# hellboywyh/pytorch-kaldi-CGS

Hardware: AMD Instinct MI355X
Metric: acoustic frames/sec (train) (higher is better)
Workload: dtype bf16; 1 GPU; TIMIT_baselines MLP 440-5x1024-{1928,48} (TIMIT_MLP_fmllr.cfg), batch_size_train=128, dropout 0.15, SGD body + RMSprop heads; global_batch=128, parallelism=dp1, chunk_frames_per_rank=225345

## Files before the change

### pytorch-kaldi-cgs_amd/csrc/pkc_gemm.hip

```cpp
#include "pkc_gemm_big.h"
#include "pkc_ops.h"
#include "pkc_optim.h"

namespace pkc {

typedef __attribute__((ext_vector_type(8))) __bf16 bf16x8;
typedef __attribute__((ext_vector_type(16))) float f32x16;

constexpr int BM = 64, BN = 64, BK = 32, NT = 256;

template <int PREC>
struct Lds;
template <>
struct Lds<PKC_PREC_FP32> {
  using T = float;
  static constexpr int LD = BK + 4;
  static constexpr int LO = 0;
  float a[BM * LD];
  float b[BN * LD];
};
template <>
struct Lds<PKC_PREC_BF16> {
  using T = __bf16;
  static constexpr int LD = BK + 8;
// ... 11 lines not shown
  __bf16 al[BM * LD];
  __bf16 bl[BN * LD];
};

template <typename T, int LO>
__device__ __forceinline__ void put(T* __restrict__ s, int i, float v) {
  const T hv = (T)v;
  s[i] = hv;
  if constexpr (LO > 0) s[i + LO] = (T)(v - (float)hv);
}

__device__ __forceinline__ int swz4(int row, int c4) { return (c4 + (row >> 2)) & 7; }

template <bool KC, bool VEC>
struct Stage {
  float v[8];
  __device__ __forceinline__ void load(const float* __restrict__ P, int64_t ld, int r0, int rmax,
                                       int k0, int kend) {
    const int t = threadIdx.x;
    if (VEC) {
#pragma unroll
      for (int i = 0; i < 2; ++i) {
        const int idx = t + NT * i;
        int r, k;
        if (KC) { r = idx >> 3; k = (idx & 7) * 4; }
        else { k = idx >> 4; r = (idx & 15) * 4; }
        const bool ok = (r0 + r < rmax) && (k0 + k < kend);
        const int rr = min(r0 + r, rmax - (KC ? 1 : 4));
        const int kk = min(k0 + k, kend - (KC ? 4 : 1));
        const float4 x = KC ? *reinterpret_cast<const float4*>(P + (int64_t)rr * ld + kk)
                            : *reinterpret_cast<const float4*>(P + (int64_t)kk * ld + rr);
        v[4 * i + 0] = ok ? x.x : 0.f;
        v[4 * i + 1] = ok ? x.y : 0.f;
        v[4 * i + 2] = ok ? x.z : 0.f;
        v[4 * i + 3] = ok ? x.w : 0.f;
      }
    } else {
#pragma unroll
      for (int i = 0; i < 8; ++i) {
        const int idx = t + NT * i;
        int r, k;
        if (KC) { r = idx >> 5; k = idx & 31; }
        else { k = idx >> 6; r = idx & 63; }
        const bool ok = (r0 + r < rmax) && (k0 + k < kend);
        const int rr = min(r0 + r, rmax - 1);
        const int kk = min(k0 + k, kend - 1);
        const float x = KC ? P[(int64_t)rr * ld + kk] : P[(int64_t)kk * ld + rr];
        v[i] = ok ? x : 0.f;
      }
    }
  }
  struct Base {
    const float* p[2];
    bool ok[2];
  };
  __device__ __forceinline__ static Base lane_base(const void* __restrict__ Pv, int64_t ld, int r0,
                                                   int rmax) {
    const float* P = reinterpret_cast<const float*>(Pv);
    const int t = threadIdx.x;
    Base b;
#pragma unroll
    for (int i = 0; i < 2; ++i) {
      const int r = KC ? (t >> 3) + 32 * i : (t & 15) * 4;
      const int rr = min(r0 + r, rmax - (KC ? 1 : 4));
      b.p[i] = KC ? P + (int64_t)rr * ld : P + rr;
      b.ok[i] = r0 + r < rmax;
    }
    return b;
  }
  __device__ __forceinline__ void load_at(const Base& b, int ld, int k0, int kend) {
    const int t = threadIdx.x;
#pragma unroll
    for (int i = 0; i < 2; ++i) {
      const int k = KC ? (t & 7) * 4 : (t >> 4) + 16 * i;
      const bool ok = b.ok[i] && (k0 + k < kend);
      const int kk = min(k0 + k, kend - (KC ? 4 : 1));
      const float4 x = KC ? *reinterpret_cast<const float4*>(b.p[i] + kk)
                          : *reinterpret_cast<const float4*>(b.p[i] + (int64_t)kk * ld);
      v[4 * i + 0] = ok ? x.x : 0.f;
      v[4 * i + 1] = ok ? x.y : 0.f;
      v[4 * i + 2] = ok ? x.z : 0.f;
      v[4 * i + 3] = ok ? x.w : 0.f;
    }
  }
  template <typename T, int LD, int LO = 0>
  __device__ __forceinline__ void store(T* __restrict__ s) const {
    const int t = threadIdx.x;
    if (VEC) {
#pragma unroll
      for (int i = 0; i < 2; ++i) {
        const int idx = t + NT * i;
        if (KC) {
          const int r = idx >> 3, k = (idx & 7) * 4;
#pragma unroll
          for (int j = 0; j < 4; ++j) put<T, LO>(s, r * LD + k + j, v[4 * i + j]);
        } else {
          const int k = idx >> 4, r = (idx & 15) * 4;
          if constexpr (sizeof(T) == 4) {
#pragma unroll
            for (int j = 0; j < 4; ++j)
              s[(r + j) * LD + 4 * swz4(r + j, k >> 2) + (k & 3)] = (T)v[4 * i + j];
          } else {
#pragma unroll
            for (int j = 0; j < 4; ++j) put<T, LO>(s, (r + j) * LD + k, v[4 * i + j]);
          }
        }
      }
    } else {
#pragma unroll
      for (int i = 0; i < 8; ++i) {
        const int idx = t + NT * i;
        if (KC) {
          const int r = idx >> 5, k = idx & 31;
          put<T, LO>(s, r * LD + k, v[i]);
        } else {
          const int k = idx >> 6, r = idx & 63;
          if constexpr (sizeof(T) == 4) s[r * LD + 4 * swz4(r, k >> 2) + (k & 3)] = (T)v[i];
          else put<T, LO>(s, r * LD + k, v[i]);
        }
      }
    }
  }
};

__device__ __forceinline__ int tr_off_s(int k, int c) { return 128 * k + 16 * (c ^ (((k >> 1) & 1) << 2)); }

__device__ __forceinline__ bf16x8 tr_frag_s(const char* __restrict__ s, int rb, int kb, int lane) {
  typedef short v4s __attribute__((ext_vector_type(4)));
  typedef short v8s __attribute__((ext_vector_type(8)));
  typedef __attribute__((address_space(3))) v4s lv4s;
  const int q = (lane & 15) >> 2, p = lane & 3;
  const int row = rb + 16 * ((lane >> 4) & 1) + 4 * p;
  const int k0 = kb + 8 * (lane >> 5) + q;
  const v4s lo = __builtin_amdgcn_ds_read_tr16_b64_v4i16(
      (lv4s*)(s + tr_off_s(k0, row >> 3) + 8 * (p & 1)));
  const v4s hi = __builtin_amdgcn_ds_read_tr16_b64_v4i16(
      (lv4s*)(s + tr_off_s(k0 + 4, row >> 3) + 8 * (p & 1)));
  const v8s w = __builtin_shufflevector(lo, hi, 0, 1, 2, 3, 4, 5, 6, 7);
  return __builtin_bit_cast(bf16x8, w);
}

__device__ __forceinline__ bf16x8 ld8h(const __bf16* p) { return *reinterpret_cast<const bf16x8*>(p); }
__device__ __forceinline__ bf16x8 zero8h() {
  bf16x8 z;
#pragma unroll
  for (int j = 0; j < 8; ++j) z[j] = (__bf16)0.f;
  return z;
}

template <bool KC, bool VEC>
struct StageH {
  bf16x8 v;
  __device__ __forceinline__ void load(const __bf16* __restrict__ P, int64_t ld, int r0, int rmax,
                                       int k0, int kend) {
    const int t = threadIdx.x;
    int r, k;
    if (KC) { r = t >> 2; k = (t & 3) * 8; }
    else { k = t >> 3; r = (t & 7) * 8; }
    if (VEC) {
      const bool ok = (r0 + r < rmax) && (k0 + k < kend);
      const int rr = min(r0 + r, rmax - (KC ? 1 : 8));
      const int kk = min(k0 + k, kend - (KC ? 8 : 1));
      const bf16x8 x = KC ? ld8h(P + (int64_t)rr * ld + kk) : ld8h(P + (int64_t)kk * ld + rr);
      v = ok ? x : zero8h();
    } else {
#pragma unroll
      for (int j = 0; j < 8; ++j) {
        const int rj = KC ? r : r + j, kj = KC ? k + j : k;
        const bool ok = (r0 + rj < rmax) && (k0 + kj < kend);
        const int rr = min(r0 + rj, rmax - 1), kk = min(k0 + kj, kend - 1);
        const __bf16 x = KC ? P[(int64_t)rr * ld + kk] : P[(int64_t)kk * ld + rr];
        v[j] = ok ? x : (__bf16)0.f;
      }
    }
  }
  struct Base {
    const __bf16* p;
    bool ok;
  };
  __device__ __forceinline__ static Base lane_base(const void* __restrict__ Pv, int64_t ld, int r0,
                                                   int rmax) {
    const __bf16* P = reinterpret_cast<const __bf16*>(Pv);
    const int t = threadIdx.x;
    const int r = KC ? t >> 2 : (t & 7) * 8;
    const int rr = min(r0 + r, rmax - (KC ? 1 : 8));
    return Base{KC ? P + (int64_t)rr * ld : P + rr, r0 + r < rmax};
  }
  __device__ __forceinline__ void load_at(const Base& b, int ld, int k0, int kend) {
    const int t = threadIdx.x;
    const int k = KC ? (t & 3) * 8 : t >> 3;
    const bool ok = b.ok && (k0 + k < kend);
    const int kk = min(k0 + k, kend - (KC ? 8 : 1));
    const bf16x8 x = KC ? ld8h(b.p + kk) : ld8h(b.p + (int64_t)kk * ld);
    v = ok ? x : zero8h();
  }
  template <typename T, int LD, int LO = 0>
  __device__ __forceinline__ void store(T* __restrict__ s) const {
    static_assert(LO == 0, "bf16-stored operands have no tail");
    const int t = threadIdx.x;
    if (KC) {
      const int r = t >> 2, k = (t & 3) * 8;
      *reinterpret_cast<bf16x8*>(&s[r * LD + k]) = v;
    } else {
      const int k = t >> 3, r = (t & 7) * 8;
      *reinterpret_cast<bf16x8*>(reinterpret_cast<char*>(s) + tr_off_s(k, r >> 3)) = v;
    }
  }
};

template <bool BIN, bool KC, bool VEC>
struct StageSel {
  using T = Stage<KC, VEC>;
  using E = float;
};
template <bool KC, bool VEC>
struct StageSel<true, KC, VEC> {
  using T = StageH<KC, VEC>;
  using E = __bf16;
};

template <int PREC, bool AKC, bool BKC, bool ATR = false, bool BTR = false>
__device__ __forceinline__ void mfma_tile(const Lds<PREC>& sm, int wm, int wn, int r, int h,
                                          f32x16& acc) {
  constexpr int LD = Lds<PREC>::LD;
  const int ra = wm * 32 + r, rb = wn * 32 + r;
  if constexpr (PREC == PKC_PREC_FP32) {
    const float4* pa = reinterpret_cast<const float4*>(&sm.a[ra * LD + 16 * h]);
    const float4* pb = reinterpret_cast<const float4*>(&sm.b[rb * LD + 16 * h]);
    float av[16], bv[16];
#pragma unroll
    for (int q = 0; q < 4; ++q) {
      float4 x, y;
      if constexpr (AKC) x = pa[q];
      else x = *reinterpret_cast<const float4*>(&sm.a[ra * LD + 4 * swz4(ra, 4 * h + q)]);
      if constexpr (BKC) y = pb[q];
      else y = *reinterpret_cast<const float4*>(&sm.b[rb * LD + 4 * swz4(rb, 4 * h + q)]);
      av[4 * q] = x.x; av[4 * q + 1] = x.y; av[4 * q + 2] = x.z; av[4 * q + 3] = x.w;
      bv[4 * q] = y.x; bv[4 * q + 1] = y.y; bv[4 * q + 2] = y.z; bv[4 * q + 3] = y.w;
    }
#pragma unroll
    for (int kk = 0; kk < 16; ++kk)
      acc = __builtin_amdgcn_mfma_f32_32x32x2f32(av[kk], bv[kk], acc, 0, 0, 0);
  } else if constexpr (PREC == PKC_PREC_BF16X3) {
#pragma unroll
    for (int t = 0; t < 2; ++t) {
      const int ia = (wm * 32 + r) * LD + 16 * t + 8 * h, ib = (wn * 32 + r) * LD + 16 * t + 8 * h;
      const bf16x8 av = *reinterpret_cast<const bf16x8*>(&sm.a[ia]);
      const bf16x8 bv = *reinterpret_cast<const bf16x8*>(&sm.b[ib]);
      const bf16x8 al = *reinterpret_cast<const bf16x8*>(&sm.al[ia]);
      const bf16x8 bl = *reinterpret_cast<const bf16x8*>(&sm.bl[ib]);
      acc = __builtin_amdgcn_mfma_f32_32x32x16_bf16(av, bl, acc, 0, 0, 0);
      acc = __builtin_amdgcn_mfma_f32_32x32x16_bf16(al, bv, acc, 0, 0, 0);
      acc = __builtin_amdgcn_mfma_f32_32x32x16_bf16(av, bv, acc, 0, 0, 0);
    }
  } else {
    const int lane = threadIdx.x & 63;
#pragma unroll
    for (int t = 0; t < 2; ++t) {
      bf16x8 av, bv;
      if constexpr (ATR) av = tr_frag_s(reinterpret_cast<const char*>(sm.a), wm * 32, 16 * t, lane);
      else av = *reinterpret_cast<const bf16x8*>(&sm.a[(wm * 32 + r) * LD + 16 * t + 8 * h]);
      if constexpr (BTR) bv = tr_frag_s(reinterpret_cast<const char*>(sm.b), wn * 32, 16 * t, lane);
      else bv = *reinterpret_cast<const bf16x8*>(&sm.b[(wn * 32 + r) * LD + 16 * t + 8 * h]);
      acc = __builtin_amdgcn_mfma_f32_32x32x16_bf16(av, bv, acc, 0, 0, 0);
    }
  }
}

template <int PREC>
__device__ __forceinline__ void tile_colstats64(const f32x16& acc, Lds<PREC>& sm, int m0, int n0,
                                                int by, int M, int N, int wm, int wn, int r, int h,
                                                const float* __restrict__ bias,
                                                float* __restrict__ part) {
  float* red = reinterpret_cast<float*>(&sm);
  const int nv = min(BM, M - m0);
  const int cl = wn * 32 + r;
  __syncthreads();
  float sum = 0.f;
#pragma unroll
  for (int reg = 0; reg < 16; ++reg) {
    const int rl = wm * 32 + (reg & 3) + 8 * (reg >> 2) + 4 * h;
    sum += rl < nv ? acc[reg] : 0.f;
  }
  sum += __shfl_xor(sum, 32);
  if (h == 0) red[wm * BN + cl] = sum;
  __syncthreads();
  const float mean = (red[cl] + red[BN + cl]) / (float)nv;
  float q = 0.f;
#pragma unroll
  for (int reg = 0; reg < 16; ++reg) {
    const int rl = wm * 32 + (reg & 3) + 8 * (reg >> 2) + 4 * h;
    const float d = acc[reg] - mean;
    q += rl < nv ? d * d : 0.f;
  }
  q += __shfl_xor(q, 32);
  if (h == 0) red[2 * BN + wm * BN + cl] = q;
  __syncthreads();
  const int col = n0 + cl;
  if (wm != 0 || h != 0 || col >= N) return;
  part[(int64_t)by * 2 * N + col] = mean + (bias ? bias[col] : 0.f);
  part[(int64_t)by * 2 * N + N + col] = red[2 * BN + cl] + red[3 * BN + cl];
}

template <int PREC, bool AKC, bool BKC, bool VEC, int DEPTH, bool BIN, bool STATS = false>
__device__ __forceinline__ void gemm_body(Lds<PREC>& sm, int bx, int by, int bz, int M, int N, int K,
                                          const void* __restrict__ Av, int64_t lda,
                                          const void* __restrict__ Bv, int64_t ldb,
                                          float* __restrict__ C, int64_t ldc, int kchunk,
                                          int64_t slab_stride, const float* __restrict__ bias = nullptr,
                                          float* __restrict__ part = nullptr) {
  using SA = typename StageSel<BIN, AKC, VEC>::T;
  using SB = typename StageSel<BIN, BKC, VEC>::T;
  const auto* A = reinterpret_cast<const typename StageSel<BIN, AKC, VEC>::E*>(Av);
  const auto* B = reinterpret_cast<const typename StageSel<BIN, BKC, VEC>::E*>(Bv);
  constexpr int LD = Lds<PREC>::LD;
  const int n0 = bx * BN, m0 = by * BM;
  const int kbeg = bz * kchunk;
  const int kend = min(K, kbeg + kchunk);
  const int lane = threadIdx.x & 63, wave = threadIdx.x >> 6;
  const int wm = wave >> 1, wn = wave & 1;
  const int r = lane & 31, h = lane >> 5;

  f32x16 acc;
#pragma unroll
  for (int i = 0; i < 16; ++i) acc[i] = 0.f;

  SA sa[DEPTH];
  SB sb[DEPTH];
  bool done = false;
  if constexpr (VEC) {
    const int nk = (kend - kbeg + BK - 1) / BK;
    if (kbeg < kend && nk <= DEPTH) {
      const typename SA::Base ab = SA::lane_base(A, lda, m0, M);
      const typename SB::Base bb = SB::lane_base(B, ldb, n0, N);
#pragma unroll
      for (int d = 0; d < DEPTH; ++d) {
        if (d >= nk) break;
        sa[d].load_at(ab, (int)lda, kbeg + d * BK, kend);
        sb[d].load_at(bb, (int)ldb, kbeg + d * BK, kend);
      }
#pragma unroll
      for (int d = 0; d < DEPTH; ++d) {
        if (d >= nk) break;
        __syncthreads();
        sa[d].template store<typename Lds<PREC>::T, LD, Lds<PREC>::LO>(sm.a);
        sb[d].template store<typename Lds<PREC>::T, LD, Lds<PREC>::LO>(sm.b);
        __syncthreads();
        mfma_tile<PREC, AKC, BKC, BIN && !AKC, BIN && !BKC>(sm, wm, wn, r, h, acc);
      }
      done = true;
    }
  }
  if constexpr (VEC) {
    if (!done && kbeg < kend) {
      const typename SA::Base ab = SA::lane_base(A, lda, m0, M);
      const typename SB::Base bb = SB::lane_base(B, ldb, n0, N);
#pragma unroll
      for (int d = 0; d < DEPTH; ++d) {
        sa[d].load_at(ab, (int)lda, kbeg + d * BK, kend);
        sb[d].load_at(bb, (int)ldb, kbeg + d * BK, kend);
      }
      for (int kt = kbeg; kt < kend; kt += DEPTH * BK) {
#pragma unroll
        for (int d = 0; d < DEPTH; ++d) {
          __syncthreads();
          sa[d].template store<typename Lds<PREC>::T, LD, Lds<PREC>::LO>(sm.a);
          sb[d].template store<typename Lds<PREC>::T, LD, Lds<PREC>::LO>(sm.b);
          __syncthreads();
          const int kn = kt + (d + DEPTH) * BK;
          sa[d].load_at(ab, (int)lda, kn, kend);
          sb[d].load_at(bb, (int)ldb, kn, kend);
          mfma_tile<PREC, AKC, BKC, BIN && !AKC, BIN && !BKC>(sm, wm, wn, r, h, acc);
        }
      }
      done = true;
    }
  }
  if (!done && kbeg < kend) {
#pragma unroll
    for (int d = 0; d < DEPTH; ++d) {
      sa[d].load(A, lda, m0, M, kbeg + d * BK, kend);
      sb[d].load(B, ldb, n0, N, kbeg + d * BK, kend);
    }
    for (int kt = kbeg; kt < kend; kt += DEPTH * BK) {
#pragma unroll
      for (int d = 0; d < DEPTH; ++d) {
        __syncthreads();
        sa[d].template store<typename Lds<PREC>::T, LD, Lds<PREC>::LO>(sm.a);
        sb[d].template store<typename Lds<PREC>::T, LD, Lds<PREC>::LO>(sm.b);
        __syncthreads();
        const int kn = kt + (d + DEPTH) * BK;
        sa[d].load(A, lda, m0, M, kn, kend);
        sb[d].load(B, ldb, n0, N, kn, kend);
        mfma_tile<PREC, AKC, BKC, BIN && !AKC, BIN && !BKC>(sm, wm, wn, r, h, acc);
      }
    }
  }
  const int col = n0 + wn * 32 + r;
  const int row0 = m0 + wm * 32 + 4 * h;
  if (col < N) {
    float* Cr = C + (int64_t)bz * slab_stride + (int64_t)row0 * ldc + col;
    const int ldci = (int)ldc;
#pragma unroll
    for (int reg = 0; reg < 16; ++reg) {
      const int dr = (reg & 3) + 8 * (reg >> 2);
      if (row0 + dr < M) Cr[dr * ldci] = acc[reg];
    }
  }
  if constexpr (STATS) tile_colstats64<PREC>(acc, sm, m0, n0, by, M, N, wm, wn, r, h, bias, part);
}

template <int PREC, bool AKC, bool BKC, bool VEC, int DEPTH, bool BIN, bool SPARSE = true>
__device__ __forceinline__ void gemm_body_sparse(Lds<PREC>& sm, int bx, int by, int bz, int M, int N, int K,
                                          const void* __restrict__ Av, int64_t lda,
                                          const void* __restrict__ Bv, int64_t ldb,
                                          float* __restrict__ C, int64_t ldc, int kchunk,
                                          int64_t slab_stride,
                                          const int32_t* __restrict__ klist = nullptr) {
  using SA = typename StageSel<BIN, AKC, VEC>::T;
  using SB = typename StageSel<BIN, BKC, VEC>::T;
  const auto* A = reinterpret_cast<const typename StageSel<BIN, AKC, VEC>::E*>(Av);
  const auto* B = reinterpret_cast<const typename StageSel<BIN, BKC, VEC>::E*>(Bv);
  constexpr int LD = Lds<PREC>::LD;
  const int n0 = bx * BN, m0 = by * BM;
  const int kbeg = SPARSE ? 0 : bz * kchunk;
  const int kend = SPARSE ? K : min(K, kbeg + kchunk);
  const int nkt = SPARSE ? klist[0] : (kend - kbeg + BK - 1) / BK;
  auto k0_of = [&](int i) {
    if constexpr (SPARSE) return i < nkt ? klist[1 + i] * BK : kend;
    else return kbeg + i * BK;
  };
  const int lane = threadIdx.x & 63, wave = threadIdx.x >> 6;
  const int wm = wave >> 1, wn = wave & 1;
  const int r = lane & 31, h = lane >> 5;

  f32x16 acc;
#pragma unroll
  for (int i = 0; i < 16; ++i) acc[i] = 0.f;

  SA sa[DEPTH];
  SB sb[DEPTH];
  if (nkt > 0) {
#pragma unroll
    for (int d = 0; d < DEPTH; ++d) {
      const int k0 = k0_of(d);
      sa[d].load(A, lda, m0, M, k0, kend);
      sb[d].load(B, ldb, n0, N, k0, kend);
    }
    for (int i0 = 0; i0 < nkt; i0 += DEPTH) {
#pragma unroll
      for (int d = 0; d < DEPTH; ++d) {
        __syncthreads();
        sa[d].template store<typename Lds<PREC>::T, LD, Lds<PREC>::LO>(sm.a);
        sb[d].template store<typename Lds<PREC>::T, LD, Lds<PREC>::LO>(sm.b);
        __syncthreads();
        const int kn = k0_of(i0 + d + DEPTH);
        sa[d].load(A, lda, m0, M, kn, kend);
        sb[d].load(B, ldb, n0, N, kn, kend);
        mfma_tile<PREC, AKC, BKC, BIN && !AKC, BIN && !BKC>(sm, wm, wn, r, h, acc);
      }
    }
  }
  const int col = n0 + wn * 32 + r;
  float* Cz = C + (int64_t)bz * slab_stride;
  if (col < N) {
#pragma unroll
    for (int reg = 0; reg < 16; ++reg) {
      const int row = m0 + wm * 32 + (reg & 3) + 8 * (reg >> 2) + 4 * h;
      if (row < M) Cz[(int64_t)row * ldc + col] = acc[reg];
    }
  }
}

template <int PREC, bool AKC, bool BKC, int DEPTH, bool BIN>
__global__ __launch_bounds__(NT) void gemm_stats_kernel(int M, int N, int K,
                                                        const void* __restrict__ A, int64_t lda,
                                                        const void* __restrict__ B, int64_t ldb,
                                                        float* __restrict__ C, int64_t ldc,
                                                        const float* __restrict__ bias,
                                                        float* __restrict__ part) {
  __shared__ Lds<PREC> sm;
  gemm_body<PREC, AKC, BKC, true, DEPTH, BIN, true>(sm, blockIdx.x, blockIdx.y, 0, M, N, K, A, lda,
                                                    B, ldb, C, ldc, ((K + BK - 1) / BK) * BK, 0,
                                                    bias, part);
}

template <int PREC, bool AKC, bool BKC, bool VEC, int DEPTH, bool BIN>
__global__ __launch_bounds__(NT) void gemm_kernel(int M, int N, int K, const void* __restrict__ A,
                                                  int64_t lda, const void* __restrict__ B,
                                                  int64_t ldb, float* __restrict__ C, int64_t ldc,
                                                  int kchunk, int64_t slab_stride) {
  __shared__ Lds<PREC> sm;
  gemm_body<PREC, AKC, BKC, VEC, DEPTH, BIN>(sm, blockIdx.x, blockIdx.y, blockIdx.z, M, N, K, A, lda,
                                             B, ldb, C, ldc, kchunk, slab_stride);
}

__device__ __forceinline__ void xcd_tile(int& bx, int& by, int& bz) {
  const int nx = gridDim.x, ny = gridDim.y;
  const int nwg = nx * ny * gridDim.z;
  int id = blockIdx.x + nx * (blockIdx.y + ny * blockIdx.z);
  if (nwg >= 16 && nwg <= 256) {
    const int xcd = id % 8, q = nwg / 8, r = nwg % 8;
    id = (xcd < r ? xcd * (q + 1) : r * (q + 1) + (xcd - r) * q) + id / 8;
  }
  bx = id % nx;
  by = (id / nx) % ny;
  bz = id / (nx * ny);
}

template <int NB, bool AKC, bool BKC, bool STATS>
__global__ __launch_bounds__(big::NT) void gemm_glds_kernel(int M, int N, int K,
                                                           const void* __restrict__ A, int64_t lda,
                                                           const void* __restrict__ B, int64_t ldb,
                                                           float* __restrict__ C, int64_t ldc,
                                                           int kchunk, int64_t slab_stride,
                                                           const float* __restrict__ bias,
                                                           float* __restrict__ part) {
  __shared__ __attribute__((aligned(16))) char lds[big::gl_lds_bytes<NB>()];
  int bx, by, bz;
  xcd_tile(bx, by, bz);
  big::body_glds<NB, AKC, BKC, STATS>(lds, bx, by, bz, M, N, K, A, lda, B, ldb, C, ldc, kchunk,
                                      slab_stride, bias, part);
}

template <int PREC, bool BIN, bool AKC, bool BKC, bool STATS>
__global__ __launch_bounds__(big::NT) void gemm_big_kernel(int M, int N, int K,
                                                          const void* __restrict__ A, int64_t lda,
                                                          const void* __restrict__ B, int64_t ldb,
                                                          float* __restrict__ C, int64_t ldc,
                                                          int kchunk, int64_t slab_stride,
                                                          const float* __restrict__ bias,
                                                          float* __restrict__ part) {
  __shared__ __attribute__((aligned(16))) char lds[big::lds_bytes<PREC>()];
  int bx, by, bz;
  xcd_tile(bx, by, bz);
  big::body<PREC, BIN, AKC, BKC, STATS>(lds, bx, by, bz, M, N, K, A, lda, B, ldb, C, ldc, kchunk,
                                        slab_stride, bias, part);
}

constexpr int GMAX = 8;
struct GroupProb {
  int kind;
  int code;
  int M, N, K, kchunk, tn, tmn, wg0;
  const void* A; int64_t lda; const void* B; int64_t ldb; float* C; int64_t ldc; int64_t slab;
  const void* X1; void* X2; void* X3;
  const int32_t* ktiles; int kmax;
  int bnb;
};
constexpr int GBNB = 2;
struct GroupArgs {
  GroupProb p[GMAX];
  int n;
  OptSegK seg[PKC_OPT_SEGS_MAX];
  big::BnEpi bnb[GBNB];
};

template <int PREC, bool BIN, bool BIG, bool SP, bool SUM, int GD, bool VO>
__device__ __forceinline__ void grouped_body(const GroupArgs& g) {
  union alignas(16) Shm {
    Lds<PREC> t;
    char big[BIG ? big::lds_bytes<PREC>() : 16];
  };
  __shared__ Shm shm;
  Lds<PREC>& sm = shm.t;
  char* lds = shm.big;
  int i = 0;
#pragma unroll
  for (int j = 1; j < GMAX; ++j)
    if (j < g.n && (int)blockIdx.x >= g.p[j].wg0) i = j;
  const GroupProb& p = g.p[i];
  const int local = blockIdx.x - p.wg0;
  if (p.kind == PKC_OP_COLSUM) {
    colsum_body(p.M, p.N, reinterpret_cast<const float*>(p.A), p.C, local * 64);
    return;
  }
  if constexpr (SUM) {
    if (p.kind == PKC_OP_SLABSUM) {
      slabsum_body(p.M, p.N, reinterpret_cast<const float*>(p.A), p.slab, p.C,
                   (int64_t)local * 1024, p.code != 0);
      return;
    }
  }
  if (p.kind == PKC_OP_OPTIM) {
    if (p.code) {
      int j = p.K;
#pragma unroll
      for (int u = 1; u < PKC_OPT_SEGS_MAX; ++u) {
        const int jj = min(p.K + u, PKC_OPT_SEGS_MAX - 1);
        if (u < p.N && local >= g.seg[jj].begin) j = jj;
      }
      const OptSegK& sg = g.seg[j];
      optim_seg_wg(reinterpret_cast<const pkc_opt_tensor*>(p.A), sg, local - sg.begin);
      return;
    }
    optim_wg(reinterpret_cast<const pkc_opt_tensor*>(p.A), reinterpret_cast<const int32_t*>(p.B),
             local);
    return;
  }
  if (p.kind == PKC_OP_GATHER) {
    gather_row_body(reinterpret_cast<const float*>(p.A), p.lda, p.N,
                    reinterpret_cast<const int32_t*>(p.B), (int)p.ldb, p.M, p.slab,
                    reinterpret_cast<const int64_t*>(p.X1), p.C, reinterpret_cast<int32_t*>(p.X2),
                    reinterpret_cast<__bf16*>(p.X3), p.code != 0, local);
    return;
  }
  if (p.kind == PKC_OP_LOSS) {
    loss_finalize_body(p.M, reinterpret_cast<const float* const*>(p.A),
                       reinterpret_cast<const float*>(p.B), p.N, reinterpret_cast<const float*>(p.X1),
                       p.C, reinterpret_cast<float*>(p.X2), reinterpret_cast<int64_t*>(p.X3));
    return;
  }
  const int bz = local / p.tmn, rem = local % p.tmn;
  const int by = rem / p.tn, bx = rem % p.tn;
  if constexpr (BIG) {
    if (p.code >= 8 && p.bnb >= 0) {
      big::body<PREC, BIN, true, false, false, true>(lds, bx, by, bz, p.M, p.N, p.K, p.A, p.lda, p.B,
                                                     p.ldb, p.C, p.ldc, p.kchunk, p.slab, nullptr,
                                                     nullptr, &g.bnb[p.bnb < GBNB ? p.bnb : 0]);
      return;
    }
    if (p.code >= 8) {
#define PKC_BB(AK, BK_)                                                                          \
  big::body<PREC, BIN, AK, BK_>(lds, bx, by, bz, p.M, p.N, p.K, p.A, p.lda, p.B, p.ldb, p.C, p.ldc, \
                                p.kchunk, p.slab)
      switch (p.code & 6) {
        case 6: PKC_BB(true, true); break;
        case 4: PKC_BB(true, false); break;
        case 2: PKC_BB(false, true); break;
        default: PKC_BB(false, false); break;
      }
#undef PKC_BB
      return;
    }
  }
  if (SP && p.ktiles) {
    const int32_t* kl = p.ktiles + (int64_t)bx * (p.kmax + 1);
#define PKC_GS(AK, BK_, V)                                                                      \
  gemm_body_sparse<PREC, AK, BK_, V, 4, BIN>(sm, bx, by, bz, p.M, p.N, p.K, p.A, p.lda, p.B,     \
                                            p.ldb, p.C, p.ldc, p.kchunk, p.slab, kl)
    switch (p.code & 7) {
      case 7: PKC_GS(true, true, true); break;
      case 6: PKC_GS(true, true, false); break;
      case 5: PKC_GS(true, false, true); break;
      default: PKC_GS(true, false, false); break;
    }
#undef PKC_GS
    return;
  }
#define PKC_GB(AK, BK_, V)                                                                      \
  gemm_body<PREC, AK, BK_, V, GD, BIN>(sm, bx, by, bz, p.M, p.N, p.K, p.A, p.lda, p.B, p.ldb, p.C, \
                                      p.ldc, p.kchunk, p.slab)
  if constexpr (VO) {
    switch (p.code) {
      case 7: PKC_GB(true, true, true); break;
      case 5: PKC_GB(true, false, true); break;
      case 1: PKC_GB(false, false, true); break;
      default: PKC_GB(false, true, true); break;
    }
    return;
  }
  switch (p.code) {
    case 7: PKC_GB(true, true, true); break;
    case 6: PKC_GB(true, true, false); break;
    case 5: PKC_GB(true, false, true); break;
    case 4: PKC_GB(true, false, false); break;
    case 1: PKC_GB(false, false, true); break;
    case 0: PKC_GB(false, false, false); break;
    case 3: PKC_GB(false, true, true); break;
    default: PKC_GB(false, true, false); break;
  }
#undef PKC_GB
}

template <int PREC, bool BIN, bool BIG, bool SP = false, bool SUM = false>
__global__ __launch_bounds__(NT) void gemm_grouped_kernel(GroupArgs g) {
  grouped_body<PREC, BIN, BIG, SP, SUM, 4, false>(g);
}

template <int PREC, bool BIN>
__global__ __launch_bounds__(NT) __attribute__((amdgpu_waves_per_eu(4, 4)))
void gemm_grouped_vo4_kernel(GroupArgs g) {
  grouped_body<PREC, BIN, false, false, false, 4, true>(g);
}

template <int PREC, bool AKC, bool BKC, bool VEC, bool BIN>
static int launch(int M, int N, int K, const void* A, int64_t lda, const void* B, int64_t ldb,
                  float* C, int64_t ldc, int splits, int64_t slab, hipStream_t s) {
  int kchunk = (K + splits - 1) / splits;
  kchunk = ((kchunk + BK - 1) / BK) * BK;
  dim3 grid((N + BN - 1) / BN, (M + BM - 1) / BM, splits);
  hipLaunchKernelGGL((gemm_kernel<PREC, AKC, BKC, VEC, BIN ? 8 : 4, BIN>), grid, dim3(NT), 0, s, M,
                     N, K, A, lda, B, ldb, C, ldc, kchunk, slab);
  PKC_LAUNCH_CHECK("pkc_gemm");
  return PKC_OK;
}

template <int PREC, bool BIN, bool STATS = false>
static int launch_big(int akc, int bkc, int M, int N, int K, const void* A, int64_t lda,
                      const void* B, int64_t ldb, float* C, int64_t ldc, int splits, int64_t slab,
                      hipStream_t s, const float* bias = nullptr, float* part = nullptr) {
  constexpr int BKB = big::Cfg<PREC, BIN>::BK;
  int kchunk = (K + splits - 1) / splits;
  kchunk = ((kchunk + BKB - 1) / BKB) * BKB;
  dim3 grid((N + big::TN - 1) / big::TN, (M + big::TM - 1) / big::TM, splits);
  if (BIN && K % 64 == 0 && (int64_t)grid.x * grid.y * grid.z <= 256) {
#define PKC_L(AK, BK_)                                                                          \
  hipLaunchKernelGGL((gemm_glds_kernel<3, AK, BK_, STATS>), grid, dim3(big::NT), 0, s, M, N, K, A, \
                     lda, B, ldb, C, ldc, kchunk, slab, bias, part)
    if (akc && bkc) PKC_L(true, true);
    else if (akc) PKC_L(true, false);
    else if (bkc) PKC_L(false, true);
    else PKC_L(false, false);
#undef PKC_L
    PKC_LAUNCH_CHECK("pkc_gemm (128x128 LDS-DMA)");
    return PKC_OK;
  }
#define PKC_L(AK, BK_)                                                                          \
  hipLaunchKernelGGL((gemm_big_kernel<PREC, BIN, AK, BK_, STATS>), grid, dim3(big::NT), 0, s, M, N, \
                     K, A, lda, B, ldb, C, ldc, kchunk, slab, bias, part)
  if (akc && bkc) PKC_L(true, true);
  else if (akc) PKC_L(true, false);
  else if (bkc) PKC_L(false, true);
  else PKC_L(false, false);
#undef PKC_L
  PKC_LAUNCH_CHECK("pkc_gemm (128x128)");
  return PKC_OK;
}

template <int PREC, bool BIN>
static int dispatch(int akc, int bkc, bool vec, int M, int N, int K, const void* A, int64_t lda,
                    const void* B, int64_t ldb, float* C, int64_t ldc, int splits, int64_t slab,
                    hipStream_t s) {
#define PKC_G(AK, BK_, V) \
  return launch<PREC, AK, BK_, V, BIN>(M, N, K, A, lda, B, ldb, C, ldc, splits, slab, s)
  if (akc && bkc) { if (vec) PKC_G(true, true, true); PKC_G(true, true, false); }
  if (akc && !bkc) { if (vec) PKC_G(true, false, true); PKC_G(true, false, false); }
  if (!akc && !bkc) { if (vec) PKC_G(false, false, true); PKC_G(false, false, false); }
  if (vec) PKC_G(false, true, true);
  PKC_G(false, true, false);
#undef PKC_G
}

constexpr int BIG_MIN_TILES = 160, BIG_MIN_TILES_GROUPED = 32, BIG_MIN_K_GROUPED = 1024;
static bool big_enabled() {
  static const bool on = env_flag("PKC_GEMM_BIG", true);
  return on;
}

}

extern "C" int pkc_gemm_pick_splits(int M, int N, int K) {
  using namespace pkc;
  const int tiles = ((M + BM - 1) / BM) * ((N + BN - 1) / BN);
  const int ktiles = (K + BK - 1) / BK;
  int s = (256 + tiles - 1) / tiles;
  s = s < 1 ? 1 : s;
  s = s > 8 ? 8 : s;
  if (s > ktiles / 2) s = ktiles / 2 > 0 ? ktiles / 2 : 1;
  int kchunk = (((K + s - 1) / s + BK - 1) / BK) * BK;
  return (K + kchunk - 1) / kchunk;
}

extern "C" int pkc_gemm(int prec, int a_kcontig, int b_kcontig, int M, int N, int K,
                        const void* A, int64_t lda, const void* B, int64_t ldb, float* C,
                        int64_t ldc, int splits, int64_t slab_stride, void* stream) {
  using namespace pkc;
  PKC_CHECK_ARG(M >= 0 && N >= 0 && K >= 0, "pkc_gemm: negative shape");
  PKC_CHECK_ARG(prec == PKC_PREC_FP32 || prec == PKC_PREC_BF16 || prec == PKC_PREC_BF16IN ||
                    prec == PKC_PREC_BF16X3,
                "pkc_gemm: bad precision %d", prec);
  if (M == 0 || N == 0) return PKC_OK;
  PKC_CHECK_ARG(A && B && C, "pkc_gemm: null operand");
  PKC_CHECK_ARG(lda > 0 && ldb > 0 && lda < (1ll << 31) && ldb < (1ll << 31),
                "pkc_gemm: leading dimensions must be in [1, 2^31)");
  PKC_CHECK_ARG(ldc >= N && ldc < (1ll << 26), "pkc_gemm: ldc must be in [N, 2^26)");
  if (splits <= 0) splits = pkc_gemm_pick_splits(M, N, K);
  PKC_CHECK_ARG(splits == 1 || slab_stride >= (int64_t)M * ldc, "pkc_gemm: slab_stride too small");
  const int e = prec == PKC_PREC_BF16IN ? 8 : 4;
  const bool vec = ((uintptr_t)A % 16 == 0) && ((uintptr_t)B % 16 == 0) && lda % e == 0 &&
                   ldb % e == 0 && (a_kcontig ? K % e == 0 : M % e == 0) &&
                   (b_kcontig ? K % e == 0 : N % e == 0);
  if (big_enabled() && big::eligible(prec, a_kcontig, b_kcontig, M, N, K, A, lda, B, ldb, BIG_MIN_TILES)) {
    if (prec == PKC_PREC_FP32)
      return launch_big<PKC_PREC_FP32, false>(a_kcontig, b_kcontig, M, N, K, A, lda, B, ldb, C, ldc,
                                              splits, slab_stride, S(stream));
    if (prec == PKC_PREC_BF16IN)
      return launch_big<PKC_PREC_BF16, true>(a_kcontig, b_kcontig, M, N, K, A, lda, B, ldb, C, ldc,
                                             splits, slab_stride, S(stream));
    if (prec == PKC_PREC_BF16X3)
      return launch_big<PKC_PREC_BF16X3, false>(a_kcontig, b_kcontig, M, N, K, A, lda, B, ldb, C,
                                                ldc, splits, slab_stride, S(stream));
    return launch_big<PKC_PREC_BF16, false>(a_kcontig, b_kcontig, M, N, K, A, lda, B, ldb, C, ldc,
                                            splits, slab_stride, S(stream));
  }
  if (prec == PKC_PREC_FP32)
    return dispatch<PKC_PREC_FP32, false>(a_kcontig, b_kcontig, vec, M, N, K, A, lda, B, ldb, C,
                                          ldc, splits, slab_stride, S(stream));
  if (prec == PKC_PREC_BF16X3)
    return dispatch<PKC_PREC_BF16X3, false>(a_kcontig, b_kcontig, vec, M, N, K, A, lda, B, ldb, C,
                                            ldc, splits, slab_stride, S(stream));
  if (prec == PKC_PREC_BF16IN)
    return dispatch<PKC_PREC_BF16, true>(a_kcontig, b_kcontig, vec, M, N, K, A, lda, B, ldb, C,
                                         ldc, splits, slab_stride, S(stream));
  return dispatch<PKC_PREC_BF16, false>(a_kcontig, b_kcontig, vec, M, N, K, A, lda, B, ldb, C, ldc,
                                        splits, slab_stride, S(stream));
}

extern "C" int pkc_gemm_bnbwd_ok(int prec, int a_kcontig, int b_kcontig, int M, int N, int K,
                                 const void* A, int64_t lda, const void* B, int64_t ldb) {
  using namespace pkc;
  if (!(prec == PKC_PREC_FP32 || prec == PKC_PREC_BF16 || prec == PKC_PREC_BF16IN) || M <= 0 ||
      N <= 0 || K <= 0 || lda <= 0 || ldb <= 0 || lda >= (1ll << 31) || ldb >= (1ll << 31) ||
      !a_kcontig || b_kcontig)
    return 0;
  return big_enabled() && big::eligible(prec, a_kcontig, b_kcontig, M, N, K, A, lda, B, ldb,
                                        BIG_MIN_TILES_GROUPED, BIG_MIN_K_GROUPED) ? 128 : 0;
}

extern "C" int pkc_gemm_grouped_tile(int prec, int a_kcontig, int b_kcontig, int M, int N, int K,
                                     const void* A, int64_t lda, const void* B, int64_t ldb) {
  using namespace pkc;
  if (M <= 0 || N <= 0 || K <= 0 || lda <= 0 || ldb <= 0) return 64;
  return big_enabled() &&
                 big::eligible(prec, a_kcontig, b_kcontig, M, N, K, A, lda, B, ldb,
                               BIG_MIN_TILES_GROUPED, BIG_MIN_K_GROUPED) ? 128 : 64;
}

extern "C" int pkc_gemm_colstats_ok(int prec, int a_kcontig, int b_kcontig, int M, int N, int K,
                                    const void* A, int64_t lda, const void* B, int64_t ldb) {
  using namespace pkc;
  if (!(prec == PKC_PREC_FP32 || prec == PKC_PREC_BF16 || prec == PKC_PREC_BF16IN ||
        prec == PKC_PREC_BF16X3) || M <= 0 ||
      N <= 0 || K <= 0 || lda <= 0 || ldb <= 0 || lda >= (1ll << 31) || ldb >= (1ll << 31))
    return 0;
  if (big_enabled() &&
      big::eligible(prec, a_kcontig, b_kcontig, M, N, K, A, lda, B, ldb, BIG_MIN_TILES))
    return 128;
  const int e = prec == PKC_PREC_BF16IN ? 8 : 4;
  const bool vec = ((uintptr_t)A % 16 == 0) && ((uintptr_t)B % 16 == 0) && lda % e == 0 &&
                   ldb % e == 0 && (a_kcontig ? K % e == 0 : M % e == 0) &&
                   (b_kcontig ? K % e == 0 : N % e == 0);
  return vec ? 64 : 0;
}

extern "C" int pkc_gemm_colstats(int prec, int a_kcontig, int b_kcontig, int M, int N, int K,
                                 const void* A, int64_t lda, const void* B, int64_t ldb, float* C,
                                 int64_t ldc, const float* bias, float* part, void* stream) {
  using namespace pkc;
  PKC_CHECK_ARG(A && B && C && part && ldc >= N, "pkc_gemm_colstats: bad arguments");
  const int rows = pkc_gemm_colstats_ok(prec, a_kcontig, b_kcontig, M, N, K, A, lda, B, ldb);
  PKC_CHECK_ARG(rows > 0, "pkc_gemm_colstats: %dx%dx%d (prec %d): no column-statistics body", M, N,
                K, prec);
  PKC_CHECK_ARG(ldc < (1ll << 26), "pkc_gemm_colstats: ldc must be below 2^26");
  if (rows == 64) {
    dim3 grid((N + BN - 1) / BN, (M + BM - 1) / BM, 1);
#define PKC_CS(P, BIN, AK, BK_)                                                                  \
  hipLaunchKernelGGL((gemm_stats_kernel<P, AK, BK_, BIN ? 8 : 4, BIN>), grid, dim3(NT), 0, S(stream), \
                     M, N, K, A, lda, B, ldb, C, ldc, bias, part)
#define PKC_CSO(P, BIN)                                                                          \
  do {                                                                                         \
    if (a_kcontig && b_kcontig) PKC_CS(P, BIN, true, true);                                    \
    else if (a_kcontig) PKC_CS(P, BIN, true, false);                                           \
    else if (b_kcontig) PKC_CS(P, BIN, false, true);                                           \
    else PKC_CS(P, BIN, false, false);                                                         \
  } while (0)
    if (prec == PKC_PREC_FP32) PKC_CSO(PKC_PREC_FP32, false);
    else if (prec == PKC_PREC_BF16X3) PKC_CSO(PKC_PREC_BF16X3, false);
    else if (prec == PKC_PREC_BF16IN) PKC_CSO(PKC_PREC_BF16, true);
    else PKC_CSO(PKC_PREC_BF16, false);
#undef PKC_CSO
#undef PKC_CS
    PKC_LAUNCH_CHECK("pkc_gemm_colstats (64x64)");
    return PKC_OK;
  }
  if (prec == PKC_PREC_FP32)
    return launch_big<PKC_PREC_FP32, false, true>(a_kcontig, b_kcontig, M, N, K, A, lda, B, ldb, C,
                                                  ldc, 1, 0, S(stream), bias, part);
  if (prec == PKC_PREC_BF16IN)
    return launch_big<PKC_PREC_BF16, true, true>(a_kcontig, b_kcontig, M, N, K, A, lda, B, ldb, C,
                                                 ldc, 1, 0, S(stream), bias, part);
  if (prec == PKC_PREC_BF16X3)
    return launch_big<PKC_PREC_BF16X3, false, true>(a_kcontig, b_kcontig, M, N, K, A, lda, B, ldb,
                                                    C, ldc, 1, 0, S(stream), bias, part);
  return launch_big<PKC_PREC_BF16, false, true>(a_kcontig, b_kcontig, M, N, K, A, lda, B, ldb, C,
                                                ldc, 1, 0, S(stream), bias, part);
}

extern "C" int pkc_gemm_grouped(int prec, const pkc_gemm_problem* probs, int n, void* stream) {
  using namespace pkc;
  PKC_CHECK_ARG(probs && n >= 1 && n <= GMAX, "pkc_gemm_grouped: 1..%d problems", GMAX);
  PKC_CHECK_ARG(prec == PKC_PREC_FP32 || prec == PKC_PREC_BF16 || prec == PKC_PREC_BF16IN ||
                    prec == PKC_PREC_BF16X3,
                "pkc_gemm_grouped: bad precision %d", prec);
  GroupArgs g;
  memset(&g, 0, sizeof(g));
  int wg = 0, k = 0, nseg = 0, nbnb = 0;
  bool any_big = false, any_sparse = false, any_sum = false, all_vec = true;
  const int e = prec == PKC_PREC_BF16IN ? 8 : 4;
  for (int i = 0; i < n; ++i) any_sparse |= probs[i].kind == PKC_OP_GEMM && probs[i].ktiles != nullptr;
  for (int i = 0; i < n; ++i) {
    const pkc_gemm_problem& q = probs[i];
    if (q.kind == PKC_OP_OPTIM) {
      const pkc_opt_seg* sg = reinterpret_cast<const pkc_opt_seg*>(q.X1);
      const bool direct = sg && q.N >= 1 && nseg + q.N <= PKC_OPT_SEGS_MAX;
      PKC_CHECK_ARG(q.M > 0 && q.A && (q.B || direct), "pkc_gemm_grouped: optimizer op %d arguments",
                    i);
      GroupProb& p = g.p[k++];
      memset(&p, 0, sizeof(p));
      p.kind = q.kind;
      p.A = q.A; p.B = q.B;
      p.wg0 = wg;
      if (direct) {
        int c = 0;
        for (int j = 0; j < q.N; ++j) {
          PKC_CHECK_ARG(sg[j].nchunks > 0 && sg[j].chunk0 >= 0 && sg[j].tensor >= 0 && sg[j].p &&
                            sg[j].g && sg[j].n > (int64_t)(sg[j].chunk0 + sg[j].nchunks - 1) * OPT_CHUNK,
                        "pkc_gemm_grouped: optimizer op %d segment %d", i, j);
          OptSegK& d = g.seg[nseg + j];
          d.p = sg[j].p; d.g = sg[j].g; d.s1 = sg[j].s1; d.s2 = sg[j].s2; d.s3 = sg[j].s3;
          d.mask = sg[j].mask; d.qout = sg[j].qout; d.bout = sg[j].bout; d.n = sg[j].n;
          d.tensor = sg[j].tensor; d.chunk0 = sg[j].chunk0; d.begin = c;
          c += sg[j].nchunks;
          d.end = c;
        }
        PKC_CHECK_ARG(c == q.M, "pkc_gemm_grouped: optimizer op %d: segments hold %d chunks, M = %d",
                      i, c, q.M);
        p.code = 1; p.K = nseg; p.N = q.N;
        nseg += q.N;
      }
      wg += q.M;
      continue;
    }
    if (q.kind == PKC_OP_SLABSUM) {
      PKC_CHECK_ARG(q.M >= 1 && q.N >= 0 && q.A && q.C && (q.M == 1 || q.slab_stride >= q.N),
                    "pkc_gemm_grouped: slab-sum op %d arguments", i);
      if (q.N == 0) continue;
      GroupProb& p = g.p[k++];
      memset(&p, 0, sizeof(p));
      p.kind = q.kind;
      p.M = q.M; p.N = q.N; p.A = q.A; p.C = q.C; p.slab = q.slab_stride;
      p.code = ((uintptr_t)q.A % 16 == 0 && (uintptr_t)q.C % 16 == 0 && q.slab_stride % 4 == 0 &&
                q.N % 4 == 0) ? 1 : 0;
      p.wg0 = wg;
      wg += (q.N + 1023) / 1024;
      any_sum = true;
      continue;
    }
    if (q.kind == PKC_OP_GATHER) {
      PKC_CHECK_ARG(q.M > 0 && q.N > 0 && q.A && q.B && q.C && q.X1 && q.X2 && q.slab_stride > 0 &&
                        q.ldb >= 0 && q.ldb <= 256 && q.lda >= q.N,
                    "pkc_gemm_grouped: gather op %d arguments", i);
      GroupProb& p = g.p[k++];
      memset(&p, 0, sizeof(p));
      p.kind = q.kind;
      p.M = q.M; p.N = q.N; p.A = q.A; p.lda = q.lda; p.B = q.B; p.ldb = q.ldb; p.C = q.C;
      p.slab = q.slab_stride; p.X1 = q.X1; p.X2 = q.X2; p.X3 = q.X3;
      p.code = (q.N % 4 == 0 && q.lda % 4 == 0 && (uintptr_t)q.A % 16 == 0 &&
                (uintptr_t)q.C % 16 == 0 && (uintptr_t)q.X3 % 8 == 0) ? 1 : 0;
      p.wg0 = wg;
      wg += q.M;
      continue;
    }
    if (q.kind == PKC_OP_COLSUM || q.kind == PKC_OP_LOSS) {
      PKC_CHECK_ARG(q.M > 0 && q.N > 0 && q.A && q.C, "pkc_gemm_grouped: op %d arguments", i);
      PKC_CHECK_ARG(q.kind != PKC_OP_LOSS || (q.M <= 8 && q.B && q.X1),
                    "pkc_gemm_grouped: loss op %d arguments", i);
      GroupProb& p = g.p[k++];
      memset(&p, 0, sizeof(p));
      p.kind = q.kind;
      p.M = q.M; p.N = q.N; p.A = q.A; p.B = q.B; p.C = q.C; p.X1 = q.X1; p.X2 = q.X2; p.X3 = q.X3;
      p.wg0 = wg;
      wg += q.kind == PKC_OP_COLSUM ? (q.N + 63) / 64 : 1;
      continue;
    }
// ... 118 lines not shown
```

### pytorch-kaldi-cgs_amd/csrc/pkc_optim.h

```cpp
#pragma once
#include "pkc_common.h"

namespace pkc {

struct OptState {
  float p, g, s1, s2, s3, m;
};

__device__ __forceinline__ void opt_update(const pkc_opt_tensor& t, OptState& e) {
  float p = e.p;
  float g = e.g;
  if (t.wd != 0.f) g = g + t.wd * p;
  if (t.kind == PKC_OPT_SGD) {
    if (t.momentum != 0.f) {
      const float buf = (t.step <= 1) ? g : t.momentum * e.s1 + (1.f - t.dampening) * g;
      e.s1 = buf;
      g = t.nesterov ? g + t.momentum * buf : buf;
    }
    p = p + (-t.lr) * g;
  } else if (t.kind == PKC_OPT_RMSPROP) {
    const float sq = e.s1 * t.alpha + (1.f - t.alpha) * g * g;
    e.s1 = sq;
    float avg;
    if (t.centered) {
      const float ga = e.s2 * t.alpha + (1.f - t.alpha) * g;
      e.s2 = ga;
      avg = sqrtf(sq - ga * ga) + t.eps;
    } else {
      avg = sqrtf(sq) + t.eps;
    }
    if (t.momentum > 0.f) {
      const float buf = e.s3 * t.momentum + g / avg;
      e.s3 = buf;
      p = p + (-t.lr) * buf;
    } else {
      p = p + (-t.lr) * (g / avg);
    }
  } else {
    const float m = e.s1 + (g - e.s1) * (1.f - t.beta1);
    const float v = e.s2 * t.beta2 + (1.f - t.beta2) * g * g;
    e.s1 = m;
    e.s2 = v;
    const float bc1 = 1.f - powf(t.beta1, (float)t.step);
    const float bc2 = 1.f - powf(t.beta2, (float)t.step);
    float vv = v;
    if (t.amsgrad) {
      vv = fmaxf(e.s3, v);
      e.s3 = vv;
    }
    const float denom = sqrtf(vv) / sqrtf(bc2) + t.eps;
    p = p + (-(t.lr / bc1)) * (m / denom);
  }
  if (t.mask) p *= e.m;
  if (t.clampv > 0.f) p = fminf(fmaxf(p, -t.clampv), t.clampv);
  e.p = p;
}

__device__ __forceinline__ float quant_w(float p, int bits) {
  const float sc = ldexpf(1.f, bits - 1);
  const float sg = p > 0.f ? 1.f : (p < 0.f ? -1.f : 0.f);
  return ceilf(fabsf(p) * sc) / sc * sg;
}

#ifndef PKC_OPT_PER
#define PKC_OPT_PER 8
#endif
constexpr int OPT_T = 256, OPT_PER = PKC_OPT_PER, OPT_CHUNK = OPT_T * OPT_PER;

template <bool VEC, bool DIRECT = false>
__device__ __forceinline__ void optim_chunk(const pkc_opt_tensor& t, int64_t start) {
  constexpr int V = 4, NV = OPT_PER / V;
  const bool st1 = DIRECT ? t.s1 != nullptr : (t.kind != PKC_OPT_SGD || t.momentum != 0.f);
  const bool st2 = t.s2 != nullptr, st3 = t.s3 != nullptr, msk = t.mask != nullptr;
  const bool qw = DIRECT ? t.qout != nullptr : t.qbits > 0;
  if (VEC) {
    float4 P[NV], G[NV], S1[NV], S2[NV], S3[NV], MK[NV];
    int64_t idx[NV];
#pragma unroll
    for (int j = 0; j < NV; ++j) {
      idx[j] = start + ((int64_t)threadIdx.x + (int64_t)j * OPT_T) * V;
      const int64_t i = idx[j] < t.n ? idx[j] : 0;
      P[j] = *reinterpret_cast<const float4*>(t.p + i);
      G[j] = *reinterpret_cast<const float4*>(t.g + i);
      if (st1) S1[j] = *reinterpret_cast<const float4*>(t.s1 + i);
      if (st2) S2[j] = *reinterpret_cast<const float4*>(t.s2 + i);
      if (st3) S3[j] = *reinterpret_cast<const float4*>(t.s3 + i);
      if (msk) MK[j] = *reinterpret_cast<const float4*>(t.mask + i);
    }
#pragma unroll
    for (int j = 0; j < NV; ++j) {
      if (idx[j] >= t.n) break;
      float* pp = &P[j].x; float* gg = &G[j].x; float* a1 = &S1[j].x; float* a2 = &S2[j].x;
      float* a3 = &S3[j].x; float* mm = &MK[j].x;
      float4 Q;
      float* qq = &Q.x;
#pragma unroll
      for (int l = 0; l < V; ++l) {
        OptState e{pp[l], gg[l], st1 ? a1[l] : 0.f, st2 ? a2[l] : 0.f, st3 ? a3[l] : 0.f,
                   msk ? mm[l] : 1.f};
        opt_update(t, e);
        pp[l] = e.p; a1[l] = e.s1; a2[l] = e.s2; a3[l] = e.s3;
        if (qw) qq[l] = quant_w(e.p, t.qbits);
      }
      const int64_t i = idx[j];
      *reinterpret_cast<float4*>(t.p + i) = P[j];
      if (st1) *reinterpret_cast<float4*>(t.s1 + i) = S1[j];
      if (st2) *reinterpret_cast<float4*>(t.s2 + i) = S2[j];
      if (st3) *reinterpret_cast<float4*>(t.s3 + i) = S3[j];
      if (qw) *reinterpret_cast<float4*>(t.qout + i) = Q;
      if (t.bout) {
        typedef __attribute__((ext_vector_type(4))) __bf16 bf16x4;
        bf16x4 h;
        h[0] = (__bf16)P[j].x; h[1] = (__bf16)P[j].y; h[2] = (__bf16)P[j].z; h[3] = (__bf16)P[j].w;
        *reinterpret_cast<bf16x4*>(reinterpret_cast<__bf16*>(t.bout) + i) = h;
      }
    }
  } else {
    OptState e[OPT_PER];
#pragma unroll
    for (int j = 0; j < OPT_PER; ++j) {
      const int64_t i0 = start + threadIdx.x + (int64_t)j * OPT_T;
      const int64_t i = i0 < t.n ? i0 : 0;
      e[j].p = t.p[i];
      e[j].g = t.g[i];
      e[j].s1 = st1 ? t.s1[i] : 0.f;
      e[j].s2 = st2 ? t.s2[i] : 0.f;
      e[j].s3 = st3 ? t.s3[i] : 0.f;
      e[j].m = msk ? t.mask[i] : 1.f;
    }
#pragma unroll
    for (int j = 0; j < OPT_PER; ++j) {
      const int64_t i = start + threadIdx.x + (int64_t)j * OPT_T;
      if (i >= t.n) break;
      opt_update(t, e[j]);
      t.p[i] = e[j].p;
      if (st1) t.s1[i] = e[j].s1;
      if (st2) t.s2[i] = e[j].s2;
      if (st3) t.s3[i] = e[j].s3;
      if (qw) t.qout[i] = quant_w(e[j].p, t.qbits);
      if (t.bout) reinterpret_cast<__bf16*>(t.bout)[i] = (__bf16)e[j].p;
    }
  }
}

struct OptSegK {
  float* p; const float* g; float* s1; float* s2; float* s3; const float* mask; float* qout; void* bout;
  int64_t n;
  int tensor, chunk0, begin, end;
};

__device__ __forceinline__ bool optim_vec(const pkc_opt_tensor& t) {
  return (t.n % 4 == 0) && ((uintptr_t)t.p % 16 == 0) && ((uintptr_t)t.g % 16 == 0) &&
         ((uintptr_t)t.s1 % 16 == 0) && ((uintptr_t)t.s2 % 16 == 0) &&
         ((uintptr_t)t.s3 % 16 == 0) && ((uintptr_t)t.mask % 16 == 0) &&
         ((uintptr_t)t.qout % 16 == 0) && ((uintptr_t)t.bout % 8 == 0);
}

__device__ __forceinline__ void optim_seg_wg(const pkc_opt_tensor* ts, const OptSegK& sg, int chunk) {
  pkc_opt_tensor t = ts[sg.tensor];
  t.p = sg.p; t.g = sg.g; t.s1 = sg.s1; t.s2 = sg.s2; t.s3 = sg.s3; t.mask = sg.mask;
  t.qout = sg.qout; t.bout = sg.bout; t.n = sg.n;
  const int64_t start = (int64_t)(sg.chunk0 + chunk) * OPT_CHUNK;
  if (optim_vec(t)) optim_chunk<true, true>(t, start);
  else optim_chunk<false, true>(t, start);
}

__device__ __forceinline__ void optim_wg(const pkc_opt_tensor* ts, const int32_t* map, int wg) {
  const int ti = map[2 * wg];
  const int64_t start = (int64_t)map[2 * wg + 1] * OPT_CHUNK;
  const pkc_opt_tensor t = ts[ti];
  if (optim_vec(t)) optim_chunk<true>(t, start);
  else optim_chunk<false>(t, start);
}

}
```

Measured before the change: 902,900 frames/s.

## Stage GEMM epilogue through LDS for 16-byte buffer stores; widen optimizer writes

For one grouped GEMM variant (code 1 in the VO path), the output tile is staged through LDS in two half-tiles, then written as coalesced 16-byte buffer stores with a nontemporal/streaming flag, replacing scattered 4-byte column stores. The optimizer's vector path now uses raw buffer stores. It also pairs adjacent lanes' bf16 weight copies via DPP into 16-byte stores, and folds RMSprop updates into FMAs. This targets store-transaction overhead, at the cost of extra LDS barriers in the epilogue and more intricate tail handling in the bf16 copy.

```diff
diff --git a/pytorch-kaldi-cgs_amd/csrc/pkc_gemm.hip b/pytorch-kaldi-cgs_amd/csrc/pkc_gemm.hip
--- a/pytorch-kaldi-cgs_amd/csrc/pkc_gemm.hip
+++ b/pytorch-kaldi-cgs_amd/csrc/pkc_gemm.hip
@@ -337,7 +337,8 @@
   part[(int64_t)by * 2 * N + N + col] = red[2 * BN + cl] + red[3 * BN + cl];
 }
 
-template <int PREC, bool AKC, bool BKC, bool VEC, int DEPTH, bool BIN, bool STATS = false>
+template <int PREC, bool AKC, bool BKC, bool VEC, int DEPTH, bool BIN, bool STATS = false,
+          bool WIDE = false>
 __device__ __forceinline__ void gemm_body(Lds<PREC>& sm, int bx, int by, int bz, int M, int N, int K,
                                           const void* __restrict__ Av, int64_t lda,
                                           const void* __restrict__ Bv, int64_t ldb,
@@ -433,7 +434,38 @@
   }
   const int col = n0 + wn * 32 + r;
   const int row0 = m0 + wm * 32 + 4 * h;
-  if (col < N) {
+  bool wide = false;
+  if constexpr (WIDE) {
+    float* Ct = C + (int64_t)bz * slab_stride + (int64_t)m0 * ldc + n0;
+    wide = ldc % 4 == 0 && ldc <= (1 << 23) && (uintptr_t)Ct % 16 == 0 && n0 + BN <= N;
+    if (wide) {
+      constexpr int SLD = BN + 4;
+      static_assert(32 * SLD * sizeof(float) <= sizeof(Lds<PREC>), "staging half-tile exceeds LDS");
+      float* st = reinterpret_cast<float*>(&sm);
+      const int ldci = (int)ldc;
+      const int sr = threadIdx.x >> 4, sc = (threadIdx.x & 15) * 4;
+#pragma unroll
+      for (int half = 0; half < 2; ++half) {
+        __syncthreads();
+        if (wm == half) {
+#pragma unroll
+          for (int reg = 0; reg < 16; ++reg)
+            st[((reg & 3) + 8 * (reg >> 2) + 4 * h) * SLD + wn * 32 + r] = acc[reg];
+        }
+        __syncthreads();
+#pragma unroll
+        for (int i = 0; i < 2; ++i) {
+          const int rl = half * 32 + sr + 16 * i;
+          if (m0 + rl < M) {
+            const float4 v = *reinterpret_cast<const float4*>(&st[(sr + 16 * i) * SLD + sc]);
+            st16_wt(Ct + (int64_t)half * 32 * ldc, ((sr + 16 * i) * ldci + sc) * 4, v);
+          }
+        }
+      }
+      if constexpr (STATS) __syncthreads();
+    }
+  }
+  if (!wide && col < N) {
     float* Cr = C + (int64_t)bz * slab_stride + (int64_t)row0 * ldc + col;
     const int ldci = (int)ldc;
 #pragma unroll
@@ -683,14 +715,15 @@
 #undef PKC_GS
     return;
   }
-#define PKC_GB(AK, BK_, V)                                                                      \
-  gemm_body<PREC, AK, BK_, V, GD, BIN>(sm, bx, by, bz, p.M, p.N, p.K, p.A, p.lda, p.B, p.ldb, p.C, \
-                                      p.ldc, p.kchunk, p.slab)
+#define PKC_GB(AK, BK_, V) PKC_GBE(AK, BK_, V, false)
+#define PKC_GBE(AK, BK_, V, E)                                                                  \
+  gemm_body<PREC, AK, BK_, V, GD, BIN, false, E>(sm, bx, by, bz, p.M, p.N, p.K, p.A, p.lda, p.B,  \
+                                                 p.ldb, p.C, p.ldc, p.kchunk, p.slab)
   if constexpr (VO) {
     switch (p.code) {
       case 7: PKC_GB(true, true, true); break;
       case 5: PKC_GB(true, false, true); break;
-      case 1: PKC_GB(false, false, true); break;
+      case 1: PKC_GBE(false, false, true, true); break;
       default: PKC_GB(false, true, true); break;
     }
     return;
@@ -706,6 +739,7 @@
     default: PKC_GB(false, true, false); break;
   }
 #undef PKC_GB
+#undef PKC_GBE
 }
 
 template <int PREC, bool BIN, bool BIG, bool SP = false, bool SUM = false>
diff --git a/pytorch-kaldi-cgs_amd/csrc/pkc_optim.h b/pytorch-kaldi-cgs_amd/csrc/pkc_optim.h
--- a/pytorch-kaldi-cgs_amd/csrc/pkc_optim.h
+++ b/pytorch-kaldi-cgs_amd/csrc/pkc_optim.h
@@ -19,11 +19,11 @@
     }
     p = p + (-t.lr) * g;
   } else if (t.kind == PKC_OPT_RMSPROP) {
-    const float sq = e.s1 * t.alpha + (1.f - t.alpha) * g * g;
+    const float sq = __builtin_fmaf(g, (1.f - t.alpha) * g, e.s1 * t.alpha);
     e.s1 = sq;
     float avg;
     if (t.centered) {
-      const float ga = e.s2 * t.alpha + (1.f - t.alpha) * g;
+      const float ga = __builtin_fmaf(t.alpha, e.s2, (1.f - t.alpha) * g);
       e.s2 = ga;
       avg = sqrtf(sq - ga * ga) + t.eps;
     } else {
@@ -67,6 +67,14 @@
 #endif
 constexpr int OPT_T = 256, OPT_PER = PKC_OPT_PER, OPT_CHUNK = OPT_T * OPT_PER;
 
+__device__ __forceinline__ void st16_wt(void* base, unsigned off, float4 v) {
+  typedef __attribute__((ext_vector_type(4))) unsigned u32x4;
+  __builtin_amdgcn_raw_buffer_store_b128(
+      __builtin_bit_cast(u32x4, v),
+      __builtin_amdgcn_make_buffer_rsrc(base, (short)0, 0x7fffffff, 0x00020000), (int)off, 0,
+      16);
+}
+
 template <bool VEC, bool DIRECT = false>
 __device__ __forceinline__ void optim_chunk(const pkc_opt_tensor& t, int64_t start) {
   constexpr int V = 4, NV = OPT_PER / V;
@@ -87,8 +95,12 @@
       if (st3) S3[j] = *reinterpret_cast<const float4*>(t.s3 + i);
       if (msk) MK[j] = *reinterpret_cast<const float4*>(t.mask + i);
     }
+    typedef __attribute__((ext_vector_type(4))) __bf16 bf16x4;
+    typedef __attribute__((ext_vector_type(2))) int i32x2;
+    i32x2 H[NV];
 #pragma unroll
     for (int j = 0; j < NV; ++j) {
+      H[j] = i32x2{0, 0};
       if (idx[j] >= t.n) break;
       float* pp = &P[j].x; float* gg = &G[j].x; float* a1 = &S1[j].x; float* a2 = &S2[j].x;
       float* a3 = &S3[j].x; float* mm = &MK[j].x;
@@ -102,17 +114,42 @@
         pp[l] = e.p; a1[l] = e.s1; a2[l] = e.s2; a3[l] = e.s3;
         if (qw) qq[l] = quant_w(e.p, t.qbits);
       }
-      const int64_t i = idx[j];
-      *reinterpret_cast<float4*>(t.p + i) = P[j];
-      if (st1) *reinterpret_cast<float4*>(t.s1 + i) = S1[j];
-      if (st2) *reinterpret_cast<float4*>(t.s2 + i) = S2[j];
-      if (st3) *reinterpret_cast<float4*>(t.s3 + i) = S3[j];
-      if (qw) *reinterpret_cast<float4*>(t.qout + i) = Q;
-      if (t.bout) {
-        typedef __attribute__((ext_vector_type(4))) __bf16 bf16x4;
-        bf16x4 h;
-        h[0] = (__bf16)P[j].x; h[1] = (__bf16)P[j].y; h[2] = (__bf16)P[j].z; h[3] = (__bf16)P[j].w;
-        *reinterpret_cast<bf16x4*>(reinterpret_cast<__bf16*>(t.bout) + i) = h;
+      const unsigned off = (threadIdx.x + j * OPT_T) * V * 4;
+      st16_wt(t.p + start, off, P[j]);
+      if (st1) st16_wt(t.s1 + start, off, S1[j]);
+      if (st2) st16_wt(t.s2 + start, off, S2[j]);
+      if (st3) st16_wt(t.s3 + start, off, S3[j]);
+      if (qw) st16_wt(t.qout + start, off, Q);
+      bf16x4 h;
+      h[0] = (__bf16)P[j].x; h[1] = (__bf16)P[j].y; h[2] = (__bf16)P[j].z; h[3] = (__bf16)P[j].w;
+      H[j] = __builtin_bit_cast(i32x2, h);
+    }
+    if (t.bout) {
+      static_assert(NV == 2, "the bf16 copy pairs the two vectors of adjacent lanes");
+      __bf16* bo = reinterpret_cast<__bf16*>(t.bout);
+      if ((uintptr_t)t.bout % 16 == 0) {
+        const bool odd = threadIdx.x & 1;
+        const i32x2 give = odd ? H[0] : H[1];
+        i32x2 got;
+        got[0] = __builtin_amdgcn_mov_dpp(give[0], 0xB1, 0xF, 0xF, true);
+        got[1] = __builtin_amdgcn_mov_dpp(give[1], 0xB1, 0xF, 0xF, true);
+        typedef __attribute__((ext_vector_type(4))) int i32x4;
+        if (!odd) {
+          if (idx[0] + V < t.n) {
+            st16_wt(bo + start, threadIdx.x * V * 2,
+                                __builtin_bit_cast(float4, i32x4{H[0][0], H[0][1], got[0], got[1]}));
+          } else if (idx[0] < t.n) {
+            *reinterpret_cast<i32x2*>(bo + idx[0]) = H[0];
+          }
+          if (idx[1] < t.n && idx[1] + V >= t.n) *reinterpret_cast<i32x2*>(bo + idx[1]) = H[1];
+        } else if (idx[1] < t.n) {
+          st16_wt(bo + start, (threadIdx.x - 1 + OPT_T) * V * 2,
+                              __builtin_bit_cast(float4, i32x4{got[0], got[1], H[1][0], H[1][1]}));
+        }
+      } else {
+#pragma unroll
+        for (int j = 0; j < NV; ++j)
+          if (idx[j] < t.n) *reinterpret_cast<i32x2*>(bo + idx[j]) = H[j];
       }
     }
   } else {
```

Result: faster. 932,600 frames/s, median of 6 (+3.3%).
